# albanie/mcnCrossModalEmotions

Hardware: AMD Instinct MI355X
Metric: distillation-step samples/sec (face+audio pair) (higher is better)
Workload: dtype f32; 1 GPU; BASELINE config 4 shard: frozen resnet50 teacher fwd + VGGVox student fwd/bwd/SGD; per_gpu_batch=32, global_batch=32, face=224x224x3, teacher_batch=32, spectrogram=512x300x1, parallelism=dp1, weights=random-init (seeded), parameter_server=rccl-capi, streams=teacher one batch ahead on its own stream + wgrad side stream

## Files before the change

### include/xmodal.h

```cpp
#ifndef XMODAL_H
#define XMODAL_H
#include <stddef.h>
#ifdef __cplusplus
extern "C" {
#endif

enum {
  XM_OK = 0,
  XM_EINVAL = 1,
  XM_ENOMEM = 2,
  XM_EHIP = 3,
  XM_ETOOBIG = 4,
  XM_ENOTSUP = 5
};

enum { XM_POOL_MAX = 0, XM_POOL_AVG = 1 };
enum { XM_LOSS_SOFTMAXLOG = 0, XM_LOSS_CLASSERROR = 1 };
enum { XM_AGG_MAX = 0, XM_AGG_MEAN = 1, XM_AGG_PEAK = 2 };
enum { XM_MNR_CONVERGED = 0, XM_MNR_ITERLIMIT = 1, XM_MNR_NOTPD = 2, XM_MNR_BADINPUT = 3 };
enum { XM_ROC_OK = 0, XM_ROC_NAN = 1, XM_ROC_BADINPUT = 2 };

enum { XM_FUSE_RELU = 1, XM_BN_BATCH_MOMENTS = 2, XM_FUSE_SIGMOID = 4 };

int xm_version(void);
// ... 11 lines not shown
int xm_tune_entries(int *total, int *unsaved);
int xm_workspace_reserve(size_t bytes);
size_t xm_workspace_bytes(void);
int xm_workspace_reserve_stream(size_t bytes, void *stream);
unsigned long long xm_workspace_generation(void);
int xm_out_size(int in, int pad_a, int pad_b, int f, int dilate, int stride);

int xm_nnconv_forward(const float *x, int H, int W, int C, int N, const float *f, int FH, int FW,
                      int FC, int K, const float *b, float *y, int sy, int sx, int pt, int pb,
                      int pl, int pr, int dy, int dx, void *stream);
int xm_nnconv_forward_fused(const float *x, int H, int W, int C, int N, const float *f, int FH,
                            int FW, int FC, int K, const float *b, float *y, int sy, int sx,
                            int pt, int pb, int pl, int pr, int dy, int dx, const float *scale,
                            const float *shift, const float *residual, int flags, void *stream);
int xm_nnconv_forward_gated(const float *x, int H, int W, int C, int N, const float *f, int FH, int FW,
                            int FC, int K, const float *b, float *y, int sy, int sx, int pt, int pb,
                            int pl, int pr, int dy, int dx, const float *scale, const float *shift,
                            const float *gate, const float *residual, int flags, void *stream);
int xm_nnconv_forward_strided_residual(const float *x, int H, int W, int C, int N, const float *f, int FH, int FW,
                                       int FC, int K, const float *b, float *y, int sy, int sx, int pt, int pb,
                                       int pl, int pr, int dy, int dx, const float *scale, const float *shift,
                                       const float *gate, const float *residual, int res_H, int res_W, int res_sy,
                                       int res_sx, int flags, void *stream);
int xm_nnconv_forward_moments(const float *x, int H, int W, int C, int N, const float *f, int FH, int FW,
                              int FC, int K, const float *b, float *y, int sy, int sx, int pt, int pb,
                              int pl, int pr, int dy, int dx, float epsilon, float *moments_out, void *stream);
int xm_nnconv_backward(const float *x, int H, int W, int C, int N, const float *f, int FH, int FW,
                       int FC, int K, const float *dzdy, float *dx_out, float *df_out,
                       float *db_out, int sy, int sx, int pt, int pb, int pl, int pr, int dy,
                       int dx, void *stream);
int xm_nnconv_prepare_backward(int H, int W, int C, int N, const float *f, int FH, int FW, int FC, int K,
                               int sy, int sx, int pt, int pb, int pl, int pr, int dy, int dx, void *stream);
int xm_params_changed(void);
int xm_nnconv_backward_accum(const float *x, int H, int W, int C, int N, const float *f, int FH, int FW,
                             int FC, int K, const float *dzdy, float *dx_out, float *df_out,
                             float *db_out, int sy, int sx, int pt, int pb, int pl, int pr, int dy,
                             int dx, const float *dx_accum, void *stream);
int xm_nnconv_backward_filter_bnrelupool(const float *x, int H, int W, int C, int N, int FH, int FW, int FC, int K,
                                         int sy, int sx, int pt, int pb, int pl, int pr, int dy, int dx,
                                         const float *y, const float *bn_g, const float *bn_b, const float *moments,
                                         int train, int ph, int pw, int psy, int psx, int ppt, int ppb, int ppl,
                                         int ppr, const unsigned char *argmax, const float *y_pool,
                                         const float *dzdy_pool, float *dzdf_out, float *dzdb_out, float *dg_out,
                                         float *db_out, void *stream);
int xm_nnconv_bnorm_relu_pool_forward(const float *x, int H, int W, int C, int N, const float *f, int FH, int FW, int FC,
                                      int K, const float *bias, int sy, int sx, int pt, int pb, int pl, int pr, int dy, int dx,
// ... 220 lines not shown
```

### mcncrossmodalemotions_amd/_lib.py

```python
import ctypes as C
import os

import torch

_HERE = os.path.dirname(os.path.abspath(__file__))
SO_PATH = os.environ.get("XM_LIB_PATH") or os.path.join(_HERE, "libxmodal_hip.so")

c_fp = C.c_void_p
_i, _f, _sz, _vp = C.c_int, C.c_float, C.c_size_t, C.c_void_p

SIGNATURES = {
    "xm_version": [],
    "xm_last_error": [],
    "xm_tune_load": [C.c_char_p],
    "xm_tune_save": [C.c_char_p],
    "xm_tune_entries": [C.POINTER(C.c_int), C.POINTER(C.c_int)],
    "xm_set_exec_hint": [C.c_uint],
    "xm_get_exec_hint": [],
    "xm_workspace_reserve": [_sz],
    "xm_workspace_bytes": [],
    "xm_workspace_reserve_stream": [_sz, _vp],
    "xm_workspace_generation": [],
    "xm_device_alloc": [C.POINTER(C.c_void_p), _sz],
    "xm_device_free": [_vp],
    "xm_device_upload": [_vp, _vp, _sz],
    "xm_device_download": [_vp, _vp, _sz],
    "xm_device_synchronize": [],
    "xm_out_size": [_i] * 6,
    "xm_nnconv_forward": [c_fp] + [_i] * 4 + [c_fp] + [_i] * 4 + [c_fp, c_fp] + [_i] * 8 + [_vp],
    "xm_nnconv_forward_moments": [c_fp] + [_i] * 4 + [c_fp] + [_i] * 4 + [c_fp, c_fp] + [_i] * 8 + [_f, c_fp, _vp],
    "xm_nnconv_forward_gated": [c_fp] + [_i] * 4 + [c_fp] + [_i] * 4 + [c_fp, c_fp] + [_i] * 8 +
                               [c_fp, c_fp, c_fp, c_fp, _i, _vp],
    "xm_nnconv_forward_strided_residual": [c_fp] + [_i] * 4 + [c_fp] + [_i] * 4 + [c_fp, c_fp] + [_i] * 8 +
                                          [c_fp, c_fp, c_fp, c_fp] + [_i] * 5 + [_vp],
    "xm_nnconv_forward_fused": [c_fp] + [_i] * 4 + [c_fp] + [_i] * 4 + [c_fp, c_fp] + [_i] * 8 +
                               [c_fp, c_fp, c_fp, _i, _vp],
    "xm_nnconv_backward": [c_fp] + [_i] * 4 + [c_fp] + [_i] * 4 + [c_fp, c_fp, c_fp, c_fp] +
                          [_i] * 8 + [_vp],
    "xm_nnconv_backward_accum": [c_fp] + [_i] * 4 + [c_fp] + [_i] * 4 + [c_fp, c_fp, c_fp, c_fp] +
                                [_i] * 8 + [c_fp, _vp],
    "xm_nnconv_prepare_backward": [_i] * 4 + [c_fp] + [_i] * 12 + [_vp],
    "xm_nnconv_backward_filter_bnrelupool": [c_fp] + [_i] * 16 + [c_fp, c_fp, c_fp, c_fp] + [_i] * 9 +
                                            [c_fp, c_fp, c_fp, c_fp, c_fp, c_fp, c_fp, _vp],
    "xm_stem_gram": [c_fp] + [_i] * 11 + [_vp, _vp],
    "xm_stem_gram_moments": [_vp, c_fp, c_fp, _i, _i, _i, _f, c_fp, _vp],
    "xm_nnconv_backward_filter_bnrelupool_gram": [c_fp] + [_i] * 4 + [c_fp] + [_i] * 4 + [c_fp] + [_i] * 8 +
                                                 [c_fp, c_fp] + [_i] * 9 + [c_fp, c_fp, c_fp, _vp, c_fp, c_fp, c_fp, c_fp, _vp],
    "xm_nnconv_bnorm_relu_pool_forward": [c_fp] + [_i] * 4 + [c_fp] + [_i] * 4 + [c_fp] + [_i] * 8 + [c_fp, c_fp, _f, c_fp] +
                                         [_i] * 8 + [_vp, c_fp, c_fp, c_fp, _vp],
    "xm_params_changed": [],
    "xm_nnpool_forward": [c_fp] + [_i] * 13 + [c_fp, _vp],
    "xm_nnpool_backward": [c_fp] + [_i] * 13 + [c_fp, c_fp, _vp],
    "xm_nnpool_forward_argmax": [c_fp] + [_i] * 12 + [c_fp, c_fp, _vp],
    "xm_nnpool_backward_argmax": [c_fp] + [_i] * 12 + [c_fp, c_fp, _vp],
    "xm_nnpool_global_avg_backward_accum": [c_fp, c_fp, c_fp, _i, _i, _i, _i, _vp],
    "xm_nnbnorm_forward": [c_fp] + [_i] * 4 + [c_fp, c_fp, _f, c_fp, c_fp, c_fp, _vp],
    "xm_nnbnorm_forward_fused": [c_fp] + [_i] * 4 + [c_fp, c_fp, _f, c_fp, c_fp, c_fp, _i, _vp],
# ... 134 lines not shown
```

### mcncrossmodalemotions_amd/csrc/context.cpp

```cpp
#include <cstdlib>
#include <map>
#include <string>
#include <vector>

#include "xm_common.h"

namespace xm {
bool path_on(Path p) {
  static const char *const kEnv[kPathCount] = {"XM_NO_HYBRID",      "XM_NO_HALO",        "XM_NO_SKINNY",     "XM_NO_SKINNY4",
                                               "XM_NO_STEM",        "XM_NO_STEM_WGRAD",  "XM_NO_DMA",        "XM_NO_FUSED_STATS",
                                               "XM_DGRAD_MERGE",    "XM_NO_FAST_TRANSPOSE", "XM_NO_POOL_LDS", "XM_NO_POOL_PATCH",
                                               "XM_NO_POOL_POOLED", "XM_NO_W8", "XM_NO_WGRAD_PATCH", "XM_NO_WGRAD_PATCH_S2", "XM_NO_DGRAD_S2", "XM_NO_STEM3"};
  static bool on[kPathCount];
  static bool read = false;
  if (!read) {
    for (int i = 0; i < kPathCount; ++i) on[i] = getenv(kEnv[i]) == nullptr;
    read = true;
  }
  return on[p];
}

long long env_int(const char *name, long long dflt) {
  const char *e = getenv(name);
  return (e && *e) ? atoll(e) : dflt;
// ... 48 lines not shown

static std::map<std::string, void *> g_tables;

const void *cached_device_table(const void *host, size_t bytes) {
  std::string key((const char *)host, bytes);
  auto it = g_tables.find(key);
  if (it != g_tables.end()) return it->second;
  void *d = nullptr;
  static const bool verbose = getenv("XM_WS_VERBOSE") != nullptr;
  if (verbose) fprintf(stderr, "[xm ws] new device table %zu bytes (#%zu)\n", bytes, g_tables.size());
  if (hipMalloc(&d, bytes) != hipSuccess) return nullptr;
  if (hipMemcpy(d, host, bytes, hipMemcpyHostToDevice) != hipSuccess) {
    (void)hipFree(d);
    return nullptr;
  }
  g_tables.emplace(std::move(key), d);
  return d;
}

}

extern "C" {

int xm_version(void) { return 122; }
const char *xm_last_error(void) { return xm::err_buf(); }

int xm_workspace_reserve(size_t bytes) {
  void *p;
  return xm::ws_get(bytes, &p, nullptr);
}
int xm_workspace_reserve_stream(size_t bytes, void *stream) {
  void *p;
  return xm::ws_get(bytes, &p, (hipStream_t)stream);
}
unsigned long long xm_workspace_generation(void) { return xm::g_ws_generation; }

int xm_device_alloc(void **ptr, size_t bytes) {
  if (!ptr) return xm::fail(XM_EINVAL, "device_alloc: NULL output");
  *ptr = nullptr;
  if (bytes == 0) return XM_OK;
  hipError_t e = hipMalloc(ptr, bytes);
  if (e != hipSuccess) return xm::fail(XM_ENOMEM, "hipMalloc(%zu) -> %s", bytes, hipGetErrorString(e));
  return XM_OK;
}
int xm_device_free(void *ptr) {
  if (!ptr) return XM_OK;
  hipError_t e = hipFree(ptr);
// ... 33 lines not shown
```

### mcncrossmodalemotions_amd/csrc/conv.hip

```cpp
#include <dlfcn.h>

#include <algorithm>
#include <climits>
#include <cstdlib>
#include <map>
#include <string>
#include <vector>

#include "conv_kernels.h"
#include "conv_tune.h"
#include "prof.h"

namespace xm {


__global__ void pad_filter_kernel(const float *__restrict__ f, float *__restrict__ o, int M, int R,
                                  int Rp) {
  size_t i = blockIdx.x * (size_t)blockDim.x + threadIdx.x;
  if (i >= (size_t)M * Rp) return;
  int r = (int)(i % Rp);
  size_t m = i / Rp;
  o[i] = r < R ? f[m * R + r] : 0.f;
}

// ... 1090 lines not shown
    return rc_;
  };
  const TuneKey key = tune_key_forward(0, g, a.M, a.NP, a.Rp, mode + (s.ok ? 4 : 0));
  const int ci = tune_cfg(key, pick_cfg(a.M, a.NP, a.Rp / kBK), st, gemm, a.dmaOk ? kNumCfg : kNumBaseCfg, w8_skip(a.M, a.NP));
  if (!a.rsOn && stem_ok(a, g, x, s.ok)) {
    auto arm = [&](int h) { return h ? launch_stem(stats_args(a, s, s.ok ? stem_grid(a.NP) : 0), f, g.R, st) : gemm(ci); };
    return arm(select_arm(7, key, st, 2, kOneChallenger, kHaloMargin, g_force_stem, arm));
  }
  if (!a.rsOn && stem3_ok(a, g, x, s.ok)) {
    auto arm = [&](int h) { return h ? launch_stem3(a, f, g.R, st) : gemm(ci); };
    return arm(select_arm(12, key, st, 2, kOneChallenger, kHaloMargin, g_force_stem3, arm));
  }
  ConvGemmArgs ah = a;
  const int hneed = (forced_tiling() || a.rsOn) ? 0 : halo_setup(ah, g.N);
  const bool hok[4] = {true, halo_var_ok(ah, hneed, 0), halo_var_ok(ah, hneed, 1), halo_var_ok(ah, hneed, 2)};
  auto arm = [&](int h) {
    if (!h) return gemm(ci);
    const bool carry = s.ok && halo_splits(ah, h - 1) == 1;
    return launch_halo(stats_args(ah, s, carry ? (a.NP + 127) / 128 : 0), h - 1, slab, st);
  };
  return arm(select_arm(4, key, st, 4, hok, kHaloMargin, halo_forced(hok), arm));
}

static int conv_forward(const float *x, const float *f, const float *b, float *y, const Geo &g,
                        const float *scale, const float *shift, const float *resid, int relu,
                        hipStream_t st, float *moments_out = nullptr, float eps = 0.f, const float *gate = nullptr,
                        int res_H = 0, int res_W = 0, int res_sy = 1, int res_sx = 1) {
  const bool padded = (g.pt | g.pb | g.pl | g.pr) != 0;
  const bool bigTaps = g.FH * g.FW > 63;
  if (bigTaps && padded)
    return fail(XM_ENOTSUP, "vl_nnconv: padded filters with more than 63 spatial taps (%dx%d) are not built",
                g.FH, g.FW);
  const int Rp = (g.R + kBK - 1) / kBK * kBK;
  const bool need_pad = (g.R % kBK) != 0 || ((uintptr_t)f & 15);
  const int mode = (padded || Rp != g.R) ? 1 : 0;
  const int NP = g.Ho * g.Wo * g.N;
  const size_t slabf = slab_floats(g.Kg, NP, Rp, kNumCfg, g.FH, g.FW, g.R);
  const bool dma_ok = !need_pad && mode == 0 && g.FH == 1 && g.FW == 1 && g.sy == 1 && g.sx == 1 && g.dy == 1 &&
                      g.dx == 1 && (g.H * g.W) % 4 == 0 && ((uintptr_t)x & 15) == 0 && ((uintptr_t)f & 15) == 0 &&
                      g.R % kBK == 0 && path_on(kPathDma);
  const bool want_stats = moments_out != nullptr && g.G == 1 && path_on(kPathFusedStats);
  const size_t statf = want_stats ? (size_t)2 * g.K * std::max((NP + 31) / 32, stem_grid(NP)) : 0;
  const size_t stat2 = want_stats ? (size_t)2 * g.K * 64 : 0;
  WsCarver ws;
  int rc = ws.init(WsCarver::need(need_pad ? (size_t)g.K * Rp : 0, 4) + WsCarver::need(slabf, 4) +
                       WsCarver::need(statf, 4) + WsCarver::need(stat2, 8), st);
  if (rc) return rc;
  FwdOperands o{x, f, b, scale, shift, resid, gate, y, device_taps(fwd_tap_table(g, Rp, bigTaps)), g.R, Rp, relu, bigTaps, dma_ok};
  if (!o.taps) return fail(XM_ENOMEM, "vl_nnconv: tap table allocation failed");
  if (resid) o.rH = res_H > 0 ? res_H : g.Ho, o.rW = res_W > 0 ? res_W : g.Wo, o.rsy = res_sy, o.rsx = res_sx;
  if (need_pad) {
    float *Ap = ws.take<float>((size_t)g.K * Rp);
    size_t n = (size_t)g.K * Rp;
    hipLaunchKernelGGL(pad_filter_kernel, dim3((unsigned)((n + 255) / 256)), dim3(256), 0, st, f, Ap,
                       g.K, g.R, Rp);
    XM_LAUNCH_CHECK();
    o.A = Ap;
    o.lda = Rp;
  }
  float *slab = slabf ? ws.take<float>(slabf) : nullptr;
  float *statp = statf ? ws.take<float>(statf) : nullptr;
  double *statp2 = stat2 ? ws.take<double>(stat2) : nullptr;
  bool stats_done = false;
  if (moments_out) g_last_stats_splits = 0;
  for (int grp = 0; grp < g.G; ++grp) {
    ConvGemmArgs a = forward_args(g, grp, o);
    FwdStats s{want_stats && a.vecStore && !relu && !resid, statp, 0};
    if (s.ok) a.dmaOk = 0;
    rc = forward_run(g, a, x, f, mode, slab, s, st);
    if (rc) return rc;
    if (s.ncg > 0) {
      rc = forward_stats_reduce(s, statp2, moments_out, g.K, NP, eps, st);
      if (rc) return rc;
      stats_done = true;
    }
  }
  if (moments_out && !stats_done) return bn_batch_moments(y, g.Ho, g.Wo, g.K, g.N, eps, moments_out, st);
  return XM_OK;
}

struct PrepKey {
  const float *f;
  int FH, FW, FC, K, G, sy, sx, dy, dx, pt, pl, H, W, fold;
  bool operator<(const PrepKey &o) const { return memcmp(this, &o, sizeof(PrepKey)) < 0; }
};
struct PrepEntry {
  float *buf = nullptr;
  size_t bytes = 0;
  unsigned long long version = ~0ull;
  hipEvent_t ev = nullptr;
  hipStream_t st = nullptr;
};
static std::map<PrepKey, PrepEntry> g_prep;
unsigned long long g_param_version = 1;
static PrepKey prep_key(const float *f, const Geo &g, bool fold) {
  PrepKey k;
  memset(&k, 0, sizeof k);
  k.f = f, k.FH = g.FH, k.FW = g.FW, k.FC = g.FC, k.K = g.K, k.G = g.G, k.sy = g.sy, k.sx = g.sx, k.dy = g.dy, k.dx = g.dx;
  k.pt = g.pt, k.pl = g.pl, k.H = g.H, k.W = g.W, k.fold = fold ? 1 : 0;
  return k;
// ... 527 lines not shown
    {"dgrad_s2", &g_force_dgrad_s2, norm_tri},
    {"spec_blocks", &g_spec_blocks, [](int v) { return v > 0 ? v : 0; }},
};
static const DebugSwitch *debug_switch(const char *key) {
  for (const DebugSwitch &s : kDebugSwitches)
    if (key && strcmp(key, s.name) == 0) return &s;
  return nullptr;
}

extern "C" {

int xm_debug_set(const char *key, int value) {
  if (const DebugSwitch *s = debug_switch(key)) {
    const int old = *s->value;
    *s->value = s->normalise(value);
    return old;
  }
  if (key && strcmp(key, "comm_single") == 0) return comm_force_single(value);
  return INT_MIN;
}
int xm_debug_get(const char *key) {
  if (key && strcmp(key, "num_conv_cfgs") == 0) return kNumCfg;
  if (key && strcmp(key, "conv_last_combine") == 0) return g_last_combine;
  if (key && strcmp(key, "wgrad_last_splits") == 0) return g_last_wgrad_splits;
  if (key && strcmp(key, "bias_grad_last_splits") == 0) return g_last_bias_splits;
  if (key && strcmp(key, "stats_last_splits") == 0) return g_last_stats_splits;
  if (key && strcmp(key, "dgrad_last_transpose") == 0) return g_last_dgrad_transpose;
  if (key && strcmp(key, "dgrad_last_prepared") == 0) return g_last_dgrad_prepared;
  const DebugSwitch *s = debug_switch(key);
  return s ? *s->value : INT_MIN;
}

int xm_set_exec_hint(unsigned flags) {
  if (flags & ~(unsigned)XM_EXEC_SINGLE_STREAM) return fail(XM_EINVAL, "xm_set_exec_hint: unknown flag bits 0x%x", flags);
  g_exec_hint = flags;
  return XM_OK;
}
unsigned xm_get_exec_hint(void) { return g_exec_hint; }


int xm_tune_load(const char *path) {
  return g_tune.load(path && path[0] ? path : tune_default_path().c_str());
}
int xm_tune_save(const char *path) {
  tune_load_once();
  const std::string p = path && path[0] ? std::string(path) : tune_default_path();
// ... 54 lines not shown
                             shift);
  rc = conv_forward(x, f, b, y, g, scale, shift, residual, (flags & XM_FUSE_RELU) ? 1 : 0, st, nullptr, 0.f, gate, res_H,
                    res_W, res_sy, res_sx);
  if (rc || !(flags & XM_FUSE_SIGMOID)) return rc;
  return xm_nnsigmoid(y, (size_t)g.Ho * g.Wo * g.K * g.N, nullptr, y, stream);
}

int xm_nnconv_forward_fused(const float *x, int H, int W, int C, int N, const float *f, int FH,
                            int FW, int FC, int K, const float *b, float *y, int sy, int sx,
                            int pt, int pb, int pl, int pr, int dy, int dx, const float *scale,
                            const float *shift, const float *residual, int flags, void *stream) {
  return fused_forward(x, H, W, C, N, f, FH, FW, FC, K, b, y, sy, sx, pt, pb, pl, pr, dy, dx, scale, shift, nullptr, residual,
                       0, 0, 1, 1, flags, stream);
}

int xm_nnconv_forward_strided_residual(const float *x, int H, int W, int C, int N, const float *f, int FH, int FW,
                                       int FC, int K, const float *b, float *y, int sy, int sx, int pt, int pb,
                                       int pl, int pr, int dy, int dx, const float *scale, const float *shift,
                                       const float *gate, const float *residual, int res_H, int res_W, int res_sy,
                                       int res_sx, int flags, void *stream) {
  if (residual && res_H < 1) return fail(XM_EINVAL, "vl_nnconv(fused): residual extent must be positive");
  return fused_forward(x, H, W, C, N, f, FH, FW, FC, K, b, y, sy, sx, pt, pb, pl, pr, dy, dx, scale, shift, gate, residual,
                       residual ? res_H : 0, res_W, res_sy, res_sx, flags, stream);
}

int xm_nnconv_forward_moments(const float *x, int H, int W, int C, int N, const float *f, int FH, int FW,
                              int FC, int K, const float *b, float *y, int sy, int sx, int pt, int pb,
                              int pl, int pr, int dy, int dx, float epsilon, float *moments_out, void *stream) {
  Geo g;
  int rc = make_geo(g, H, W, C, N, FH, FW, FC, K, sy, sx, pt, pb, pl, pr, dy, dx);
  if (rc) return rc;
  if (!x || !f || !y || !moments_out) return fail(XM_EINVAL, "vl_nnconv(+moments): NULL tensor");
  hipStream_t st = (hipStream_t)stream;
  if (fc_skinny_ok(g)) {
    g_last_stats_splits = 0;
    rc = fc_skinny_forward(x, f, b, y, g, 0, st);
    return rc ? rc : bn_batch_moments(y, g.Ho, g.Wo, g.K, g.N, epsilon, moments_out, st);
  }
  return conv_forward(x, f, b, y, g, nullptr, nullptr, nullptr, 0, st, moments_out, epsilon);
}

int xm_nnconv_forward_gated(const float *x, int H, int W, int C, int N, const float *f, int FH, int FW,
                            int FC, int K, const float *b, float *y, int sy, int sx, int pt, int pb,
                            int pl, int pr, int dy, int dx, const float *scale, const float *shift,
                            const float *gate, const float *residual, int flags, void *stream) {
  if (!gate) return fail(XM_EINVAL, "vl_nnconv(gated): NULL tensor");
// ... 105 lines not shown
```

### mcncrossmodalemotions_amd/csrc/conv_plan.h

```cpp
#pragma once
#include <cstddef>
#include <cstdint>
#include <vector>

namespace xm {

constexpr int kBK = 16;
constexpr int kHaloCB = 8;
constexpr int kStemHP = 520;
constexpr int kStemNV = 7;
constexpr int kStem3CS = 232;
constexpr int kSpNC = 9;
constexpr int kDgS2Rows = 96;

struct Geo {
  int H, W, C, N, FH, FW, FC, K, G, Kg, Ho, Wo, R;
  int sy, sx, pt, pb, pl, pr, dy, dx;
};

inline bool fits_i32_bytes(size_t elements) { return elements * 4 < (1ull << 31); }
inline size_t x_elements(const Geo &g) { return (size_t)g.H * g.W * g.C * g.N; }
inline size_t y_elements(const Geo &g) { return (size_t)g.Ho * g.Wo * g.K * g.N; }

struct Tap2 {
// ... 2 lines not shown
struct Tap4 {
  int off, du, dv, zero;
};

inline int x_tap(const Geo &g, int r, int *u, int *v) {
  *u = r % g.FH, *v = (r / g.FH) % g.FW;
  return 4 * (*u * g.dy + g.H * (*v * g.dx) + g.H * g.W * (r / (g.FH * g.FW)));
}
inline std::vector<Tap2> fwd_tap_table(const Geo &g, int Rp, bool all_valid) {
  std::vector<Tap2> t(Rp + 3 * kBK, Tap2{0, 63});
  for (int r = 0, u, v; r < g.R; ++r) {
    const int off = x_tap(g, r, &u, &v);
    t[r] = Tap2{off, all_valid ? 0 : u + g.FH * v};
  }
  return t;
}
inline std::vector<Tap4> wgrad_tap_table(const Geo &g, int count) {
  std::vector<Tap4> t(count, Tap4{0, -(1 << 28), 0, 0});
  for (int r = 0, u, v; r < g.R; ++r) {
    const int off = x_tap(g, r, &u, &v);
    t[r] = Tap4{off, u * g.dy, v * g.dx, 0};
  }
  return t;
}

struct DgradClass {
  int a, b, u0, ustep, nU, v0, vstep, nV, Rc, Rp, i0, hi0, PI, j0, wi0, PJ;
};

inline bool dgrad_fold_h(const Geo &g) {
  return g.Ho == 1 && g.FH > 1 && g.FH == g.H && g.pt == 0 && g.pb == 0 && g.dy == 1 && g.sy == 1;
}

inline void class_taps(int F, int d, int s, int a, int *t0, int *step, int *n) {
  *t0 = -1, *step = 1, *n = 0;
  for (int t = 0; t < F; ++t)
    if ((t * d) % s == a) {
      if (*t0 < 0) *t0 = t;
      else if (*n == 1) *step = t - *t0;
      ++*n;
    }
}

inline std::vector<DgradClass> dgrad_classes(const Geo &g, bool foldH, bool *covers_all) {
  std::vector<DgradClass> cls;
  *covers_all = true;
// ... 114 lines not shown
```

### mcncrossmodalemotions_amd/dagnn.py

```python
import os
from collections import OrderedDict

import numpy as np
import torch

from . import vl


class Param:
    def __init__(self, name, value=None, learningRate=1.0, weightDecay=1.0, trainMethod="gradient"):
        self.name = name
        self.value = value
        self.der = None
        self.learningRate = learningRate
        self.weightDecay = weightDecay
        self.trainMethod = trainMethod
        self.fanout = 0


class Var:
    def __init__(self, name):
        self.name = name
        self.value = None
        self.der = None
# ... 396 lines not shown

class DagNN:

    def __init__(self):
        self.layers = []
        self.vars = OrderedDict()
        self.params = OrderedDict()
        self.meta = {}
        self.mode = "normal"
        self.conserveMemory = True
        self.accumulateParamDers = False
        self.fuse = True
        self.fuseStats = os.environ.get("XM_NO_FUSED_STATS") is None
        self.wgradAfterDgrad = os.environ.get("XM_WGRAD_AFTER_DGRAD") is not None
        self.fuseBiasDer = os.environ.get("XM_NO_FUSED_BIASDER") is None
        self.fuseStemBackward = os.environ.get("XM_NO_FUSED_STEM_BWD") is None
        self.fuseStemGram = os.environ.get("XM_NO_STEM_GRAM") is None
        self.fuseStemForward = os.environ.get("XM_NO_STEM_FWD") is None
        self.fuseForkSums = os.environ.get("XM_NO_FORK_SUMS") is None
        self.fuseSE = os.environ.get("XM_NO_FUSED_SE") is None
        self.foldSEReduce = os.environ.get("XM_NO_SE_FOLD_FC") is None
        self.fuseSETrain = os.environ.get("XM_NO_FUSED_SE_BWD") is None
        self.stridePrune = os.environ.get("XM_STRIDE_PRUNE", "1") != "0"
        self.wgradStream = None
        self.gradHook = None
        self.markHook = None
        self.bwdHooks = {}
        self._side_pending = False
        self._training = False
        self.prepareBackward = os.environ.get("XM_NO_PREPARE") is None
        self.device = None
        self._flat = None
        self._gen = [0]
        self._plan_key = self._plan_layers = self._plan_cache = None
        self._der_consts = {}

    @property
    def paramGeneration(self):
        return self._gen[0]

    @paramGeneration.setter
    def paramGeneration(self, v):
        self._gen[0] = int(v)
        if self.device is not None:
            vl.params_changed()

# ... 47 lines not shown
            l.block.net = self
            for v in l.inputs:
                self.vars.setdefault(v, old.get(v) or Var(v))
            for v in l.outputs:
                self.vars.setdefault(v, old.get(v) or Var(v))
        for v in self.vars.values():
            v.fanin = v.fanout = 0
        for l in self.layers:
            for v in l.inputs:
                self.vars[v].fanout += 1
            for v in l.outputs:
                self.vars[v].fanin += 1
            for p in l.params:
                self.params[p].fanout += 1
        used = {p for l in self.layers for p in l.params}
        for p in list(self.params):
            if p not in used:
                del self.params[p]

    def replica(self):
        import copy
        r = DagNN()
        r.meta, r.mode, r.fuse, r.device = self.meta, self.mode, self.fuse, self.device
        r.conserveMemory, r.stridePrune = self.conserveMemory, self.stridePrune
        for l in self.layers:
            r.layers.append(_LayerRec(l.name, copy.copy(l.block), l.inputs, l.outputs, l.params))
        r.params = self.params
        r._gen = self._gen
        r.rebuild()
        for name, v in self.vars.items():
            r.vars[name].precious = v.precious
        return r

    @staticmethod
    def loadobj(s):
        from . import matfile
        return matfile.loadobj(s)

    def saveobj(self):
        from . import matfile
        return matfile.saveobj(self)

    def getLayerIndex(self, name):
        for i, l in enumerate(self.layers):
            if l.name == name:
                return i
        return None
# ... 145 lines not shown
            return None
        ps = [self.params[p] for p in rec.params]
        if any(p.fanout > 1 or p.der is None for p in ps):
            return None
        return [p.der for p in ps]

    def _set_param_der(self, name, d):
        if d is None:
            return
        p = self.params[name]
        if self._flat is not None and d is p.der:
            return
        seen = self._pending_param_ders.get(name, 0)
        self._pending_param_ders[name] = seen + 1
        if self._flat is not None:
            if seen == 0 and not self.accumulateParamDers:
                p.der.copy_(d)
            else:
                p.der.add_(d)
        else:
            p.der = d if (p.der is None or seen == 0 and not self.accumulateParamDers) else vl.sum2(p.der, d)

    def _plan(self, training):
        key = (training, self.mode, self.fuse, self.stridePrune, len(self.layers),
               tuple(n for n, v in self.vars.items() if v.precious))
        layers = [id(l) for l in self.layers]
        if self._plan_key != key or self._plan_layers != layers:
            self._plan_key, self._plan_layers, self._plan_cache = key, layers, build_plan(self, training)
        return self._plan_cache


def load_mat(path):
    from . import matfile
    return matfile.load_mat(path)


def save_mat(net, path, wrap=None):
    from . import matfile
    return matfile.save_mat(net, path, wrap)


class FlatParams:
    def __init__(self, val, der, mom, segments):
        self.val, self.der, self.mom, self.segments = val, der, mom, segments
        self.state2 = None
        self.solver_t = None


def _release_der(net, var):
    if net.conserveMemory and not var.precious:
        var.der = None


class _Step:

    reads_through_conv = False

    def __init__(self, rec, *swallowed):
        self.rec = rec
        self.recs = [rec] + [q for q in swallowed if q is not None]
        self.outputs = self.recs[-1].outputs
        made = {v for q in self.recs for v in q.outputs}
        self.reads = tuple(dict.fromkeys(v for q in self.recs for v in q.inputs if v not in made))
        self.run_stride = None

    def _stride(self):
        return self.rec.block.stride if self.run_stride is None else self.run_stride

    def _params(self, net):
        return [net.params[p].value for p in self.rec.params]

    def _values(self, net, ins):
        return self.rec.block.forward(ins, self._params(net))

    def _derivatives(self, net, ins, douts):
        return self.rec.block.backward(ins, self._params(net), douts)

    def forward(self, net):
        outs = self._values(net, [net.vars[v].value for v in self.rec.inputs])
        for v, t in zip(self.outputs, outs):
            net.vars[v].value = t

    def backward(self, net):
        r = self.rec
        douts = [net.vars[v].der for v in self.outputs]
        if all(d is None for d in douts):
            return
# ... 416 lines not shown

    def _fold(self, net):
        g, b, mom = [net.params[p].value for p in self.bn_rec.params]
        key = (g.data_ptr(), b.data_ptr(), mom.data_ptr(), g._version, b._version, mom._version,
               net.paramGeneration)
        if self._folded is None or self._folded[0] != key:
            gn, bn_, mn = vl.to_numpy(g).ravel(), vl.to_numpy(b).ravel(), vl.to_numpy(mom)
            sc = (gn / mn[:, 1]).astype(np.float32)
            sh = (bn_ - mn[:, 0] * sc).astype(np.float32)
            self._folded = (key, vl.from_numpy(sc.reshape(-1, 1), g.device),
                            vl.from_numpy(sh.reshape(-1, 1), g.device))
        return self._folded[1], self._folded[2]

    def _values(self, net, ins):
        blk, prm = self.rec.block, self._params(net)
        sc, sh = self._fold(net)
        resid = None
        if self.sum_rec is not None:
            other = [v for v in self.sum_rec.inputs if v != self.bn_rec.outputs[0]][0]
            resid = net.vars[other].value
        pruned = self.run_stride if (resid is not None and self.run_stride != (1, 1)) else None
        return [vl.vl_nnconv(ins[0], prm[0], prm[1] if blk.hasBias else None, stride=self._stride(), pad=blk.pad,
                             dilate=blk.dilate, scale=sc, shift=sh, residual=resid, residual_stride=pruned,
                             relu=self.relu_rec is not None)]

    def backward(self, net):
        raise RuntimeError("folded conv+bn steps exist only in forward-only test-mode plans")


class _SEFoldStep(_ConvFoldStep):

    reads_through_conv = False

    def __init__(self, conv_rec, bn_rec, se):
        super().__init__(conv_rec, bn_rec, None, se["relu"],
                         between=[se[k] for k in ("gp", "fc1", "relu1", "fc2", "sig", "axpy")])
        self.se = se
        self._reduce = None

    def _fold_reduce(self, net, F, bias, sc, sh, F1, b1):
        ts = [t for t in (F, bias, sc, sh, F1, b1) if t is not None]
        key = tuple(t.data_ptr() for t in ts) + tuple(t._version for t in ts) + (net.paramGeneration,)
        if self._reduce is None or self._reduce[0] != key:
            Kp, Cc = int(F.shape[2]), int(F.shape[3])
            Fm = vl.to_numpy(F).astype(np.float64).reshape(Kp, Cc, order="F")
            F1m = vl.to_numpy(F1).astype(np.float64).reshape(Cc, int(F1.shape[3]), order="F")
            scn, shn = vl.to_numpy(sc).astype(np.float64).ravel(), vl.to_numpy(sh).astype(np.float64).ravel()
# ... 163 lines not shown


def _prune_strided_boundaries(w, steps):
    head = {id(st.rec): st for st in steps}
    for st in steps:
        if not isinstance(st, _ConvFoldStep) or st.run_stride is not None or \
                not _conv_1x1(st.rec.block, unit_stride=True) or w.net.vars[st.outputs[0]].precious:
            continue
        readers = [head.get(id(c)) for c in w.consumers.get(st.outputs[0], [])]
        if not readers or any(q is None or not q.reads_through_conv or not _conv_1x1(q.rec.block) or
                              q.run_stride is not None for q in readers):
            continue
        strides = {tuple(vl._pair(q.rec.block.stride, "STRIDE")) for q in readers}
        if len(strides) != 1:
            continue
        s = strides.pop()
        if s[0] != s[1] or s[0] <= 1:
            continue
        st.run_stride = s
        for q in readers:
            q.run_stride = (1, 1)


def build_plan(net, training):
    w = _Wiring(net)
    fold = net.fuse and not training and net.mode == "test"
    steps, taken = [], set()
    for r in net.layers:
        if id(r) in taken:
            continue
        st = _fold_forward_only(w, r) if fold else None
        if st is None and net.fuse:
            st = _fuse_common(w, r) or (_se_train_head(w, r) if training else None)
        steps.append(st or _unfused(r))
        taken.update(id(q) for q in steps[-1].recs[1:])
    if net.fuse and training:
        _link_training(w, steps)
    if fold and net.stridePrune:
        _prune_strided_boundaries(w, steps)
    return steps
```

### mcncrossmodalemotions_amd/vl.py

```python
import ctypes as C

import numpy as np
import torch

from . import _lib



def _dev():
    return torch.device("cuda", torch.cuda.current_device())


XM_ENOTSUP = 5


def mat_empty(*shape, device=None):
    shape = tuple(int(s) for s in (shape[0] if len(shape) == 1 and not np.isscalar(shape[0]) else shape))
    t = torch.empty(tuple(reversed(shape)), dtype=torch.float32, device=device or _dev())
    return t.permute(*reversed(range(len(shape))))


def mat_zeros(*shape, device=None):
    t = mat_empty(*shape, device=device)
    t.zero_()
# ... 76 lines not shown
    _lib.check(_L().xm_tune_entries(C.byref(tot), C.byref(new)))
    _lib.check(_L().xm_tune_save(path.encode() if path else None))
    return int(tot.value), int(new.value)


EXEC_SINGLE_STREAM = 1


def set_exec_hint(flags):
    old = int(_L().xm_get_exec_hint())
    _lib.check(_L().xm_set_exec_hint(int(flags)))
    return old


def out_size(n, pa, pb, f, d, s):
    return _L().xm_out_size(n, pa, pb, f, d, s)




def vl_nnconv(x, f, b=None, dzdy=None, stride=1, pad=0, dilate=1, no_der_data=False,
              no_der_filters=False, no_der_biases=False, scale=None, shift=None, residual=None,
              relu=False, df_out=None, db_out=None, dx_accum=None, sigmoid=False, moments_out=None, epsilon=1e-4,
              gate=None, residual_stride=None):
    x, f = _chk(x, "X"), _chk(f, "F")
    H, W, Cc, N = _shape4(x)
    FH, FW, FC, K = _shape4(f)
    sy, sx = _pair(stride, "STRIDE")
    dy, dx = _pair(dilate, "DILATE")
    pt, pb, pl, pr = _pad4(pad)
    bb = None
    if b is not None and b.numel() > 0:
        bb = _chk(b, "B")
        if bb.numel() != K:
            raise ValueError("vl_nnconv: B has %d elements, expected %d" % (bb.numel(), K))
    L = _L()
    Ho = L.xm_out_size(H, pt, pb, FH, dy, sy)
    Wo = L.xm_out_size(W, pl, pr, FW, dx, sx)
    if dzdy is None:
        y = mat_empty(max(Ho, 0), max(Wo, 0), K, N, device=x.device)
        fused = scale is not None or residual is not None or relu or sigmoid
        if residual_stride is not None:
            if residual is None:
                raise ValueError("vl_nnconv: residual_stride without a residual")
            if moments_out is not None or sigmoid:
                raise ValueError("vl_nnconv: residual_stride cannot be combined with moments_out or sigmoid")
            rsy, rsx = _pair(residual_stride, "RESIDUAL_STRIDE")
            RH, RW, RK, RN = _shape4(_chk(residual, "RESIDUAL"))
            if [RK, RN] != [K, N]:
                raise ValueError("vl_nnconv: residual shape mismatch")
            gt = None
            if gate is not None:
                gt = _chk(gate, "GATE")
                if gt.numel() != K * N:
                    raise ValueError("vl_nnconv: GATE must be 1 x 1 x %d x %d" % (K, N))
            _lib.check(L.xm_nnconv_forward_strided_residual(
                _ptr(x), H, W, Cc, N, _ptr(f), FH, FW, FC, K, _ptr(bb), _ptr(y), sy, sx, pt, pb, pl, pr, dy, dx,
                _ptr(scale), _ptr(shift), _ptr(gt), _ptr(residual), RH, RW, rsy, rsx, 1 if relu else 0, _stream()))
        elif gate is not None:
            gt = _chk(gate, "GATE")
            if gt.numel() != K * N:
                raise ValueError("vl_nnconv: GATE must be 1 x 1 x %d x %d" % (K, N))
            if residual is not None and _shape4(_chk(residual, "RESIDUAL")) != [Ho, Wo, K, N]:
                raise ValueError("vl_nnconv: residual shape mismatch")
            _lib.check(L.xm_nnconv_forward_gated(
# ... 1446 lines not shown
```

Before: 4131 pairs/s.

## Compute only lattice pixels read by strided 1x1 consumers in folded forward

Adds a lattice-restricted conv forward that evaluates only the output pixels a downstream strided-pruned 1x1 conv will read. The plan builder tags eligible folded conv steps, reusing the existing GEMM config, split-K and hybrid planning for the smaller pixel set. This is meant to skip forward work on outputs that are never consumed. In exchange it adds a new planning path with lattice index maths, and it falls back when tuning or halo arms disagree.

```diff
diff --git a/include/xmodal.h b/include/xmodal.h
--- a/include/xmodal.h
+++ b/include/xmodal.h
@@ -57,6 +57,10 @@
                                        int pl, int pr, int dy, int dx, const float *scale, const float *shift,
                                        const float *gate, const float *residual, int res_H, int res_W, int res_sy,
                                        int res_sx, int flags, void *stream);
+int xm_nnconv_forward_lattice(const float *x, int H, int W, int C, int N, const float *f, int FH, int FW, int FC, int K,
+                              const float *b, float *y, int sy, int sx, int pt, int pb, int pl, int pr, int dy, int dx,
+                              const float *scale, const float *shift, const float *residual, int flags, int lat_y,
+                              int lat_x, void *stream);
 int xm_nnconv_forward_moments(const float *x, int H, int W, int C, int N, const float *f, int FH, int FW,
                               int FC, int K, const float *b, float *y, int sy, int sx, int pt, int pb,
                               int pl, int pr, int dy, int dx, float epsilon, float *moments_out, void *stream);
diff --git a/mcncrossmodalemotions_amd/_lib.py b/mcncrossmodalemotions_amd/_lib.py
--- a/mcncrossmodalemotions_amd/_lib.py
+++ b/mcncrossmodalemotions_amd/_lib.py
@@ -33,6 +33,8 @@
                                [c_fp, c_fp, c_fp, c_fp, _i, _vp],
     "xm_nnconv_forward_strided_residual": [c_fp] + [_i] * 4 + [c_fp] + [_i] * 4 + [c_fp, c_fp] + [_i] * 8 +
                                           [c_fp, c_fp, c_fp, c_fp] + [_i] * 5 + [_vp],
+    "xm_nnconv_forward_lattice": [c_fp] + [_i] * 4 + [c_fp] + [_i] * 4 + [c_fp, c_fp] + [_i] * 8 +
+                                 [c_fp, c_fp, c_fp, _i, _i, _i, _vp],
     "xm_nnconv_forward_fused": [c_fp] + [_i] * 4 + [c_fp] + [_i] * 4 + [c_fp, c_fp] + [_i] * 8 +
                                [c_fp, c_fp, c_fp, _i, _vp],
     "xm_nnconv_backward": [c_fp] + [_i] * 4 + [c_fp] + [_i] * 4 + [c_fp, c_fp, c_fp, c_fp] +
diff --git a/mcncrossmodalemotions_amd/csrc/context.cpp b/mcncrossmodalemotions_amd/csrc/context.cpp
--- a/mcncrossmodalemotions_amd/csrc/context.cpp
+++ b/mcncrossmodalemotions_amd/csrc/context.cpp
@@ -94,7 +94,7 @@
 
 extern "C" {
 
-int xm_version(void) { return 122; }
+int xm_version(void) { return 123; }
 const char *xm_last_error(void) { return xm::err_buf(); }
 
 int xm_workspace_reserve(size_t bytes) {
diff --git a/mcncrossmodalemotions_amd/csrc/conv.hip b/mcncrossmodalemotions_amd/csrc/conv.hip
--- a/mcncrossmodalemotions_amd/csrc/conv.hip
+++ b/mcncrossmodalemotions_amd/csrc/conv.hip
@@ -1136,6 +1136,12 @@
   return arm(select_arm(4, key, st, 4, hok, kHaloMargin, halo_forced(hok), arm));
 }
 
+static bool fwd_dma_ok(const Geo &g, const float *x, const float *f, bool need_pad, int mode) {
+  return !need_pad && mode == 0 && g.FH == 1 && g.FW == 1 && g.sy == 1 && g.sx == 1 && g.dy == 1 &&
+         g.dx == 1 && (g.H * g.W) % 4 == 0 && ((uintptr_t)x & 15) == 0 && ((uintptr_t)f & 15) == 0 &&
+         g.R % kBK == 0 && path_on(kPathDma);
+}
+
 static int conv_forward(const float *x, const float *f, const float *b, float *y, const Geo &g,
                         const float *scale, const float *shift, const float *resid, int relu,
                         hipStream_t st, float *moments_out = nullptr, float eps = 0.f, const float *gate = nullptr,
@@ -1150,9 +1156,7 @@
   const int mode = (padded || Rp != g.R) ? 1 : 0;
   const int NP = g.Ho * g.Wo * g.N;
   const size_t slabf = slab_floats(g.Kg, NP, Rp, kNumCfg, g.FH, g.FW, g.R);
-  const bool dma_ok = !need_pad && mode == 0 && g.FH == 1 && g.FW == 1 && g.sy == 1 && g.sx == 1 && g.dy == 1 &&
-                      g.dx == 1 && (g.H * g.W) % 4 == 0 && ((uintptr_t)x & 15) == 0 && ((uintptr_t)f & 15) == 0 &&
-                      g.R % kBK == 0 && path_on(kPathDma);
+  const bool dma_ok = fwd_dma_ok(g, x, f, need_pad, mode);
   const bool want_stats = moments_out != nullptr && g.G == 1 && path_on(kPathFusedStats);
   const size_t statf = want_stats ? (size_t)2 * g.K * std::max((NP + 31) / 32, stem_grid(NP)) : 0;
   const size_t stat2 = want_stats ? (size_t)2 * g.K * 64 : 0;
@@ -1190,6 +1194,155 @@
     }
   }
   if (moments_out && !stats_done) return bn_batch_moments(y, g.Ho, g.Wo, g.K, g.N, eps, moments_out, st);
+  return XM_OK;
+}
+
+struct FullExtentPlan {
+  int ci;
+  int tps;
+  int hyS, hyTps, hyP0;
+};
+static int g_last_lattice = 0;
+
+static bool full_extent_plan(const Geo &g, const ConvGemmArgs &a, const float *x, int mode, bool have_slab, hipStream_t st,
+                             FullExtentPlan &p) {
+  if (stem_ok(a, g, x, false) || stem3_ok(a, g, x, false)) return false;
+  const TuneKey key = tune_key_forward(0, g, a.M, a.NP, a.Rp, mode);
+  int ci = pick_cfg(a.M, a.NP, a.Rp / kBK);
+  const int ncfg = a.dmaOk ? kNumCfg : kNumBaseCfg;
+  if (g_force_cfg >= 0) ci = g_force_cfg < ncfg ? g_force_cfg : base_cfg(g_force_cfg);
+  else if (tune_must_measure(key, st, &ci)) return false;
+  ConvGemmArgs ah = a;
+  const int hneed = forced_tiling() ? 0 : halo_setup(ah, g.N);
+  const bool hok[4] = {true, halo_var_ok(ah, hneed, 0), halo_var_ok(ah, hneed, 1), halo_var_ok(ah, hneed, 2)};
+  if (hok[1] || hok[2] || hok[3]) {
+    int arm = halo_forced(hok);
+    if (arm < 0) {
+      TuneKey k4 = key;
+      k4.kind = 4;
+      arm = 0;
+      if (tune_must_measure(k4, st, &arm)) return false;
+      if (arm < 0 || arm >= 4 || !hok[arm]) arm = 0;
+    }
+    if (arm != 0) return false;
+  }
+  ci = a.dmaOk ? ci : base_cfg(ci);
+  int sp;
+  gemm_slab_floats(a, ci, &sp);
+  if (ci == kCfgW8 && !path_on(kPathW8)) ci = 0;
+  const Cfg &c = kCfgs[ci];
+  ConvGemmArgs t = a;
+  t.nbm = (a.M + c.bm() - 1) / c.bm(), t.nbn = (a.NP + c.bn() - 1) / c.bn(), t.nkt = a.Rp / kBK;
+  t.statPart = nullptr;
+  p.tps = (t.nkt + sp - 1) / sp;
+  p.hyS = 1, p.hyTps = 0, p.hyP0 = 0;
+  if (p.tps >= t.nkt && have_slab) {
+    int full;
+    const int hyS = hybrid_plan(t, ci, &full);
+    if (hyS > 1) {
+      p.hyTps = (t.nkt + hyS - 1) / hyS;
+      p.hyS = (t.nkt + p.hyTps - 1) / p.hyTps;
+      p.hyP0 = full / t.nbm * c.bn();
+    }
+  }
+  p.ci = !is_dma_cfg(ci) ? ci : (kCfgs[ci].tm * kCfgs[ci].tn == 1 ? 3 : base_cfg(ci));
+  return true;
+}
+
+static int launch_gemm_lattice(ConvGemmArgs a, int mode, int ci, int tps, float *slab, int p0, hipStream_t st) {
+  const Cfg &c = kCfgs[ci];
+  a.nbm = (a.M + c.bm() - 1) / c.bm();
+  a.nbn = (a.NP + c.bn() - 1) / c.bn();
+  a.nkt = a.Rp / kBK;
+  a.tilesPerSplit = std::min(tps, a.nkt);
+  const int splits = (a.nkt + a.tilesPerSplit - 1) / a.tilesPerSplit;
+  a.NPs = (a.NP + 3) & ~3;
+  a.slab = splits > 1 ? slab : nullptr;
+  a.dbgCycles = g_dbg_cycles;
+  a.hyS = 1, a.hyFull = 0, a.hyTps = 0, a.hyP0 = 0;
+  if (splits > 1 && !slab) return fail(XM_EINVAL, "vl_nnconv(lattice): split launch without a slab");
+  {
+    const double abytes = (double)a.xBytes + 4.0 * a.M * a.Rtrue + 4.0 * a.M * (double)a.NP;
+    ProfScope ps(prof_key(kProfGemm, ci * 2 + mode), 2.0 * a.M * (double)a.NP * a.Rtrue, st, abytes);
+    const dim3 grid(a.nbm * a.nbn, splits);
+    if (mode) launch_gemm_cfg<1>(ci, a, grid, st);
+    else launch_gemm_cfg<0>(ci, a, grid, st);
+  }
+  XM_LAUNCH_CHECK();
+  g_last_combine = 0;
+  if (splits > 1) {
+    a.slab += p0, a.hyP0 = p0;
+    launch_splitk_epilogue(a, splits, a.NP - p0, false, st);
+    g_last_combine = -splits;
+    XM_LAUNCH_CHECK();
+  }
+  return XM_OK;
+}
+
+static int conv_forward_lattice(const float *x, const float *f, const float *b, float *y, const Geo &g, const float *scale,
+                                const float *shift, int relu, int ly, int lx, hipStream_t st, int *ran) {
+  *ran = 0;
+  const bool padded = (g.pt | g.pb | g.pl | g.pr) != 0;
+  const bool bigTaps = g.FH * g.FW > 63;
+  if (bigTaps && padded) return XM_OK;
+  if (g.G != 1) return XM_OK;
+  const int Rp = (g.R + kBK - 1) / kBK * kBK;
+  const bool need_pad = (g.R % kBK) != 0 || ((uintptr_t)f & 15);
+  const int mode = (padded || Rp != g.R) ? 1 : 0;
+  const int NP = g.Ho * g.Wo * g.N;
+  const bool have_slab = slab_floats(g.Kg, NP, Rp, kNumCfg, g.FH, g.FW, g.R) > 0;
+  const int PI = lattice_extent(g.Ho, ly), PJ = lattice_extent(g.Wo, lx), NPl = PI * PJ * g.N;
+  FwdOperands o{x, f, b, scale, shift, nullptr, nullptr, y, nullptr, g.R, Rp, relu, bigTaps, fwd_dma_ok(g, x, f, need_pad, mode)};
+  FullExtentPlan p;
+  if (!full_extent_plan(g, forward_args(g, 0, o), x, mode, have_slab, st, p)) return XM_OK;
+  const int nkt = Rp / kBK;
+  const int z = p.hyS > 1 ? p.hyS : (nkt + p.tps - 1) / p.tps;
+  const long long cut = p.hyS > 1 ? lattice_pixels_below(p.hyP0, g.Ho, g.Wo, ly, lx) : 0;
+  const int n0 = (int)(cut / (PI * PJ));
+  const int NPz = NPl - n0 * PI * PJ;
+  const size_t slabf = z > 1 ? (size_t)z * g.Kg * ((NPz + 3) & ~3) : 0;
+  WsCarver ws;
+  int rc = ws.init(WsCarver::need(need_pad ? (size_t)g.K * Rp : 0, 4) + WsCarver::need(slabf, 4), st);
+  if (rc) return rc;
+  o.taps = device_taps(fwd_tap_table(g, Rp, bigTaps));
+  if (!o.taps) return fail(XM_ENOMEM, "vl_nnconv: tap table allocation failed");
+  if (need_pad) {
+    float *Ap = ws.take<float>((size_t)g.K * Rp);
+    const size_t n = (size_t)g.K * Rp;
+    hipLaunchKernelGGL(pad_filter_kernel, dim3((unsigned)((n + 255) / 256)), dim3(256), 0, st, f, Ap, g.K, g.R, Rp);
+    XM_LAUNCH_CHECK();
+    o.A = Ap;
+    o.lda = Rp;
+  }
+  float *slab = slabf ? ws.take<float>(slabf) : nullptr;
+  for (int grp = 0; grp < g.G; ++grp) {
+    ConvGemmArgs a = forward_args(g, grp, o);
+    a.PI = PI, a.PJ = PJ, a.NP = NPl;
+    a.divPIJ = make_fastdiv((uint32_t)(PI * PJ)), a.divPI = make_fastdiv((uint32_t)PI);
+    a.gsy = g.sy * ly, a.gsx = g.sx * lx;
+    a.osy = ly, a.osx = lx;
+    a.vecStore = 0, a.dmaOk = 0;
+    if (p.hyS <= 1) {
+      rc = launch_gemm_lattice(a, mode, p.ci, p.tps, slab, 0, st);
+      if (rc) return rc;
+      continue;
+    }
+    if (cut > 0) {
+      ConvGemmArgs a1 = a;
+      a1.NP = (int)cut;
+      rc = launch_gemm_lattice(a1, mode, p.ci, nkt, nullptr, 0, st);
+      if (rc) return rc;
+    }
+    if (cut < NPl) {
+      ConvGemmArgs a2 = a;
+      const size_t xskip = (size_t)n0 * g.H * g.W * g.C;
+      a2.X += xskip, a2.xBytes -= (unsigned)(xskip * 4), a2.Y += (size_t)n0 * a.oSampleStride;
+      a2.NP = NPz;
+      rc = launch_gemm_lattice(a2, mode, p.ci, p.hyTps, slab, (int)(cut - (long long)n0 * PI * PJ), st);
+      if (rc) return rc;
+    }
+  }
+  *ran = 1;
   return XM_OK;
 }
 
@@ -1763,6 +1916,7 @@
 int xm_debug_get(const char *key) {
   if (key && strcmp(key, "num_conv_cfgs") == 0) return kNumCfg;
   if (key && strcmp(key, "conv_last_combine") == 0) return g_last_combine;
+  if (key && strcmp(key, "conv_last_lattice") == 0) return g_last_lattice;
   if (key && strcmp(key, "wgrad_last_splits") == 0) return g_last_wgrad_splits;
   if (key && strcmp(key, "bias_grad_last_splits") == 0) return g_last_bias_splits;
   if (key && strcmp(key, "stats_last_splits") == 0) return g_last_stats_splits;
@@ -1863,6 +2017,31 @@
   if (residual && res_H < 1) return fail(XM_EINVAL, "vl_nnconv(fused): residual extent must be positive");
   return fused_forward(x, H, W, C, N, f, FH, FW, FC, K, b, y, sy, sx, pt, pb, pl, pr, dy, dx, scale, shift, gate, residual,
                        residual ? res_H : 0, res_W, res_sy, res_sx, flags, stream);
+}
+
+int xm_nnconv_forward_lattice(const float *x, int H, int W, int C, int N, const float *f, int FH, int FW, int FC, int K,
+                              const float *b, float *y, int sy, int sx, int pt, int pb, int pl, int pr, int dy, int dx,
+                              const float *scale, const float *shift, const float *residual, int flags, int lat_y,
+                              int lat_x, void *stream) {
+  Geo g;
+  int rc = make_geo(g, H, W, C, N, FH, FW, FC, K, sy, sx, pt, pb, pl, pr, dy, dx);
+  if (rc) return rc;
+  if (!x || !f || !y) return fail(XM_EINVAL, "vl_nnconv: NULL tensor");
+  if (lat_y < 1 || lat_x < 1) return fail(XM_EINVAL, "vl_nnconv(lattice): the lattice steps must be >= 1, got [%d %d]", lat_y, lat_x);
+  if ((scale == nullptr) != (shift == nullptr))
+    return fail(XM_EINVAL, "vl_nnconv(fused): scale and shift must be given together");
+  if (residual) return fail(XM_ENOTSUP, "vl_nnconv(lattice): a residual operand is not built");
+  if (flags & ~XM_FUSE_RELU) return fail(XM_ENOTSUP, "vl_nnconv(lattice): only the ReLU epilogue is built");
+  g_last_lattice = 0;
+  int ran = 0;
+  if ((lat_y > 1 || lat_x > 1) && !fc_skinny_ok(g)) {
+    rc = conv_forward_lattice(x, f, b, y, g, scale, shift, (flags & XM_FUSE_RELU) ? 1 : 0, lat_y, lat_x, (hipStream_t)stream, &ran);
+    if (rc) return rc;
+  }
+  g_last_lattice = ran;
+  if (ran) return XM_OK;
+  return fused_forward(x, H, W, C, N, f, FH, FW, FC, K, b, y, sy, sx, pt, pb, pl, pr, dy, dx, scale, shift, nullptr, nullptr, 0, 0,
+                       1, 1, flags, stream);
 }
 
 int xm_nnconv_forward_moments(const float *x, int H, int W, int C, int N, const float *f, int FH, int FW,
diff --git a/mcncrossmodalemotions_amd/csrc/conv_plan.h b/mcncrossmodalemotions_amd/csrc/conv_plan.h
--- a/mcncrossmodalemotions_amd/csrc/conv_plan.h
+++ b/mcncrossmodalemotions_amd/csrc/conv_plan.h
@@ -48,6 +48,14 @@
     t[r] = Tap4{off, u * g.dy, v * g.dx, 0};
   }
   return t;
+}
+
+inline int lattice_extent(int full, int step) { return (full - 1) / step + 1; }
+inline long long lattice_pixels_below(long long p0, int Ho, int Wo, int ly, int lx) {
+  const int PI = lattice_extent(Ho, ly), PJ = lattice_extent(Wo, lx);
+  const long long n = p0 / ((long long)Ho * Wo);
+  const int q = (int)(p0 - n * Ho * Wo), j = q / Ho, i = q % Ho;
+  return n * PI * PJ + (long long)((j + lx - 1) / lx) * PI + (j % lx == 0 ? (i + ly - 1) / ly : 0);
 }
 
 struct DgradClass {
diff --git a/mcncrossmodalemotions_amd/dagnn.py b/mcncrossmodalemotions_amd/dagnn.py
--- a/mcncrossmodalemotions_amd/dagnn.py
+++ b/mcncrossmodalemotions_amd/dagnn.py
@@ -442,6 +442,7 @@
         self.foldSEReduce = os.environ.get("XM_NO_SE_FOLD_FC") is None
         self.fuseSETrain = os.environ.get("XM_NO_FUSED_SE_BWD") is None
         self.stridePrune = os.environ.get("XM_STRIDE_PRUNE", "1") != "0"
+        self.latticePrune = os.environ.get("XM_LATTICE_PRUNE", "1") != "0"
         self.wgradStream = None
         self.gradHook = None
         self.markHook = None
@@ -535,7 +536,7 @@
         import copy
         r = DagNN()
         r.meta, r.mode, r.fuse, r.device = self.meta, self.mode, self.fuse, self.device
-        r.conserveMemory, r.stridePrune = self.conserveMemory, self.stridePrune
+        r.conserveMemory, r.stridePrune, r.latticePrune = self.conserveMemory, self.stridePrune, self.latticePrune
         for l in self.layers:
             r.layers.append(_LayerRec(l.name, copy.copy(l.block), l.inputs, l.outputs, l.params))
         r.params = self.params
@@ -727,7 +728,7 @@
             p.der = d if (p.der is None or seen == 0 and not self.accumulateParamDers) else vl.sum2(p.der, d)
 
     def _plan(self, training):
-        key = (training, self.mode, self.fuse, self.stridePrune, len(self.layers),
+        key = (training, self.mode, self.fuse, self.stridePrune, self.latticePrune, len(self.layers),
                tuple(n for n, v in self.vars.items() if v.precious))
         layers = [id(l) for l in self.layers]
         if self._plan_key != key or self._plan_layers != layers:
@@ -768,6 +769,7 @@
         made = {v for q in self.recs for v in q.outputs}
         self.reads = tuple(dict.fromkeys(v for q in self.recs for v in q.inputs if v not in made))
         self.run_stride = None
+        self.out_lattice = None
 
     def _stride(self):
         return self.rec.block.stride if self.run_stride is None else self.run_stride
@@ -1230,7 +1232,7 @@
         pruned = self.run_stride if (resid is not None and self.run_stride != (1, 1)) else None
         return [vl.vl_nnconv(ins[0], prm[0], prm[1] if blk.hasBias else None, stride=self._stride(), pad=blk.pad,
                              dilate=blk.dilate, scale=sc, shift=sh, residual=resid, residual_stride=pruned,
-                             relu=self.relu_rec is not None)]
+                             relu=self.relu_rec is not None, out_lattice=self.out_lattice)]
 
     def backward(self, net):
         raise RuntimeError("folded conv+bn steps exist only in forward-only test-mode plans")
@@ -1440,6 +1442,21 @@
             q.run_stride = (1, 1)
 
 
+def _prune_reader_lattices(w, steps):
+    head = {id(st.rec): st for st in steps}
+    for st in steps:
+        if type(st) is not _ConvFoldStep or st.sum_rec is not None or st.run_stride is not None or \
+                tuple(vl._pair(st.rec.block.stride, "STRIDE")) != (1, 1) or w.net.vars[st.outputs[0]].precious:
+            continue
+        readers = [head.get(id(c)) for c in w.consumers.get(st.outputs[0], [])]
+        if len(readers) != 1 or readers[0] is None or not readers[0].reads_through_conv:
+            continue
+        s = readers[0].run_stride
+        if s is None or s[0] != s[1] or s[0] <= 1 or not _conv_1x1(readers[0].rec.block, unit_stride=True):
+            continue
+        st.out_lattice = tuple(s)
+
+
 def build_plan(net, training):
     w = _Wiring(net)
     fold = net.fuse and not training and net.mode == "test"
@@ -1456,4 +1473,6 @@
         _link_training(w, steps)
     if fold and net.stridePrune:
         _prune_strided_boundaries(w, steps)
+        if net.latticePrune:
+            _prune_reader_lattices(w, steps)
     return steps
diff --git a/mcncrossmodalemotions_amd/vl.py b/mcncrossmodalemotions_amd/vl.py
--- a/mcncrossmodalemotions_amd/vl.py
+++ b/mcncrossmodalemotions_amd/vl.py
@@ -122,7 +122,7 @@
 def vl_nnconv(x, f, b=None, dzdy=None, stride=1, pad=0, dilate=1, no_der_data=False,
               no_der_filters=False, no_der_biases=False, scale=None, shift=None, residual=None,
               relu=False, df_out=None, db_out=None, dx_accum=None, sigmoid=False, moments_out=None, epsilon=1e-4,
-              gate=None, residual_stride=None):
+              gate=None, residual_stride=None, out_lattice=None):
     x, f = _chk(x, "X"), _chk(f, "F")
     H, W, Cc, N = _shape4(x)
     FH, FW, FC, K = _shape4(f)
@@ -140,7 +140,14 @@
     if dzdy is None:
         y = mat_empty(max(Ho, 0), max(Wo, 0), K, N, device=x.device)
         fused = scale is not None or residual is not None or relu or sigmoid
-        if residual_stride is not None:
+        if out_lattice is not None:
+            if residual is not None or gate is not None or sigmoid or moments_out is not None or residual_stride is not None:
+                raise ValueError("vl_nnconv: out_lattice takes the scale / shift / relu epilogue only")
+            lty, ltx = _pair(out_lattice, "OUT_LATTICE")
+            _lib.check(L.xm_nnconv_forward_lattice(
+                _ptr(x), H, W, Cc, N, _ptr(f), FH, FW, FC, K, _ptr(bb), _ptr(y), sy, sx, pt, pb, pl, pr, dy, dx,
+                _ptr(scale), _ptr(shift), None, 1 if relu else 0, lty, ltx, _stream()))
+        elif residual_stride is not None:
             if residual is None:
                 raise ValueError("vl_nnconv: residual_stride without a residual")
             if moments_out is not None or sigmoid:
```

Measured after the change: 4191 pairs/s, median of 6. 1.01x the previous value.
